# isds-neu/PeRCNN

Hardware: AMD Instinct MI355X
Metric: pi_block_rollout_fwd_bwd_steps_per_sec (higher is better)
Workload: dtype f32; 1 GPU; gs2d_512: gs2d 512x512, 2 species, Hc=8, T=1000 forward+backward rollout per step, dense dL/dtraj; reaction=poly, parallelism=single GPU, points=262144, T=1000

## Files before the change

### percnn_amd/csrc/pi_abi.hip

```cpp
#include <hip/hip_runtime.h>

#include <cstdint>
#include <cstdlib>
#include <chrono>
#include <cstdio>
#include <cstring>
#include <map>
#include <mutex>
#include <thread>
#include <tuple>
#include <vector>

#include "../../include/percnn_pi.h"
#include "pi_kernels.h"
#include "pi_tile2d.h"
#include "pi_stream3d.h"
#include "pi_brick3d.h"
#include "pi_res3d.h"
#include "pi_contract.h"
#include "pi_peer.h"
#include "pi_adv.h"
#include "pi_host.h"

namespace {

using pi::Geom;

struct Options {
    int block = 256;
    int vec = 0;
    int wgrad_blocks = 1024;
    int tile = 1;
    int tile_k = 4;
    int tile_nt = 512;
    int stream3d = 1;
    int tile_fuse = 1;
    int bwd_cpl = 2;
    int zc = 8;
    int overlap = 0;
    int overlap_chunk = 128;
    int fuse_wgrad = 2;
    int skip_wgrad = 0;
    int tile_xcd = 1;
    int tile_by = 0;
    int slab_fused_put_adj = 0;
    int peer_upb = 2048;
    int peer_upb_take = 0;
    int tile_persist = 2;
    int persist_handshake = 1;
    int fwd_small_half = 1;
    int adj_small_half = 1;
    int adj_small_pause = -1;
    int fwd_small_pause = -1;
    int persist_small = 1;
    int fwd_persist_per_cu = 1;
    int fwd_persist_f64 = 1;
    int adj_persist_f64 = 1;
    int fwd_persist = 1;
    int persist_split = 1;
    int persist_timeout_ms = 2000;
    int persist_first_timeout_ms = 100;
    int tile_wide = 3;
    int fwd_blocks = 0;
    int xcd_window = 0;
    int block_small = 1;
    int rz = 0;
// ... 990 lines not shown
    PI_TILE_DISPATCH(CALL_AT);
#undef CALL_AT
}

int device_cu_count()
{
    static int cu_count[16] = {};
    int dev = 0;
    if (hipGetDevice(&dev) != hipSuccess || dev < 0 || dev >= 16) return 0;
    if (!cu_count[dev]) {
        int n = 0;
        cu_count[dev] = (hipDeviceGetAttribute(&n, hipDeviceAttributeMultiprocessorCount, dev) == hipSuccess && n > 0) ? n : -1;
    }
    return cu_count[dev] > 0 ? cu_count[dev] : 0;
}

bool persist_disabled_here();
constexpr int PERSIST_BAND = 2 * (TILE_B * TILE_B - (TILE_B - 16) * (TILE_B - 16));
size_t persist_outbox_bytes(const Problem& p, int elem = 4)
{
    return (size_t)2 * (size_t)((p.n0 / TILE_B) * (p.W / TILE_B)) * PERSIST_BAND * (elem == 8 ? 16 : 8);
}

template <typename T>
bool persist_ok(const Problem& p, const unsigned char* mask, int t_top, int ngroups, hipStream_t st)
{
    if (!p.opt.tile_persist || ngroups < 2) return false;
    if (sizeof(T) != 4 && (!p.opt.adj_persist_f64 || !p.opt.persist_split)) return false;
    if (persist_disabled_here()) return false;
    if (mask && t_top >= 4096) return false;
    if (!tile_fuse_ok<T>(p) || tile_wide_for<T>(p, true) != 0 || tile_by_for(p) != TILE_B) return false;
    if (p.n0 % TILE_B || p.W % TILE_B) return false;
    const int64_t tiles = (p.n0 / TILE_B) * (p.W / TILE_B);
    const int cus = device_cu_count();
    if (tiles < 16 || cus <= 0 || tiles > cus) return false;
    hipStreamCaptureStatus cap = hipStreamCaptureStatusNone;
    if (hipStreamIsCapturing(st, &cap) != hipSuccess || cap != hipStreamCaptureStatusNone) return false;
    return true;
}

constexpr int PERSIST_SLOTS = 32;
struct PersistHost {
    volatile int slot[PERSIST_SLOTS][4];
};
struct PersistGuard {
    std::mutex mu;
// ... 294 lines not shown
    if (p.n0 % TILE_B || p.W % TILE_B) return false;
    const int64_t tiles = (p.n0 / TILE_B) * (p.W / TILE_B);
    const int cus = device_cu_count();
    if (tiles < 16 || cus <= 0 || tiles > (int64_t)cus * p.opt.fwd_persist_per_cu) return false;
    hipStreamCaptureStatus cap = hipStreamCaptureStatusNone;
    if (st && (hipStreamIsCapturing(st, &cap) != hipSuccess || cap != hipStreamCaptureStatusNone)) return false;
    return true;
}

template <typename T>
hipError_t launch_fwd_persist(T* frame_t0, int ngroups, const T* P, const Problem& p, hipStream_t st)
{
    constexpr int K = 4, NT = 512;
    pi_host::Resident r;
    if (!persist_enter(st, r.dev)) return hipErrorNotSupported;
    pi::TileGeom g = make_tile_geom(p, TILE_B);
    const unsigned grid = (unsigned)((p.n0 / TILE_B) * g.tiles_x);
    const size_t lds = pi::tile_state_bytes<T, K, TILE_B, TILE_B>() + (size_t)pi::PERSIST_SPLIT_TABLE_ROWS * NT * sizeof(int) + 16;
    const int two = (int64_t)grid > (int64_t)device_cu_count() ? 1 : 0;
    auto* k = two ? pi::pi_fwd2d_persist_kernel<T, K, TILE_B, TILE_B, NT, 2> : pi::pi_fwd2d_persist_kernel<T, K, TILE_B, TILE_B, NT, 1>;
    if (hipError_t e = allow_lds(k, lds)) return e;
    const int nb = persist_fits(k, NT, lds, r.dev);
    if (nb < 1 || (int64_t)grid > (int64_t)device_cu_count() * nb) return hipErrorCooperativeLaunchTooLarge;
    if (hipError_t e = persist_scratch(persist_outbox_bytes(p, (int)sizeof(T)), st, r)) return e;
    long frame_stride = (long)(2 * p.n);
    persist_claim(p.opt, r);
    pi::PersistArgs pa = persist_args(r, reinterpret_cast<unsigned long long*>(r.scratch + 256), reinterpret_cast<unsigned*>(r.scratch), ngroups);
    void* args[] = {(void*)&frame_t0, (void*)&frame_stride, (void*)&P, (void*)&g, (void*)&pa};
    hipError_t e;
    if (p.opt.tile_persist == 2) {
        hipLaunchKernelGGL(k, dim3(grid), dim3(NT), lds, st, frame_t0, frame_stride, P, g, pa);
        e = hipGetLastError();
    } else {
        e = hipLaunchCooperativeKernel(reinterpret_cast<const void*>(k), dim3(grid), dim3(NT), args, (unsigned)lds, st);
    }
    if (e != hipSuccess) return e;
    return persist_launched(st, r, p.opt.persist_handshake, grid, "the resident forward rollout");
}

int64_t persist_small_tiles(const Problem& p, int by) { return ((p.n0 + by - 1) / by) * ((p.W + TILE_B - 1) / TILE_B); }
size_t persist_small_outbox_bytes(const Problem& p, int elem)
{
    if (p.ndim != 2 || p.hc != 0 || elem != 4 || p.slab) return 0;
    const int by = tile_by_for(p);
    if (by >= TILE_B || persist_small_tiles(p, by) > 256) return 0;
    return align_up((size_t)2 * (size_t)persist_small_tiles(p, by) * (2 * TILE_B * by) * sizeof(unsigned long long), 256);
}

template <typename T>
bool persist_small_ok(const Problem& p, const unsigned char* mask, int t_top, int ngroups, hipStream_t st)
// ... 1678 lines not shown
    else           { if (vec == 1) PI_RSB(3, 1); else PI_RSB(3, V); }
#undef PI_RSB
    return (int)hipGetLastError();
}

}

namespace {

int apply_option(Options& o, const char* key, long value)
{
    if (!key) return PERCNN_PI_EINVAL;
    if (!std::strcmp(key, "vec")) {
        if (value != 0 && value != 1) return PERCNN_PI_EINVAL;
        o.vec = (int)value;
        return 0;
    }
    if (!std::strcmp(key, "tile")) {
        if (value < 0 || value > 2) return PERCNN_PI_EINVAL;
        o.tile = (int)value;
        return 0;
    }
    if (!std::strcmp(key, "tile_xcd")) { o.tile_xcd = value != 0; return 0; }
    if (!std::strcmp(key, "tile_by")) {
        if (value != 0 && value != 8 && value != 16 && value != 32) return PERCNN_PI_EINVAL;
        o.tile_by = (int)value;
        return 0;
    }
    if (!std::strcmp(key, "slab_fused_put_adj")) { o.slab_fused_put_adj = value != 0; return 0; }
    if (!std::strcmp(key, "peer_upb") || !std::strcmp(key, "peer_upb_take")) {
        const bool take = key[8] == '_';
        if ((value < 256 && !(take && value == 0)) || value > 65536) return PERCNN_PI_EINVAL;
        (take ? o.peer_upb_take : o.peer_upb) = (int)value;
        return 0;
    }
    if (!std::strcmp(key, "tile_persist")) {
        if (value < 0 || value > 2) return PERCNN_PI_EINVAL;
        o.tile_persist = (int)value;
        return 0;
    }
    if (!std::strcmp(key, "persist_handshake")) { o.persist_handshake = value != 0; return 0; }
    if (!std::strcmp(key, "persist_split")) { o.persist_split = value != 0; return 0; }
    if (!std::strcmp(key, "persist_small")) { if (value < 0 || value > 2) return PERCNN_PI_EINVAL; o.persist_small = (int)value; return 0; }
    if (!std::strcmp(key, "fwd_persist")) { o.fwd_persist = value != 0; return 0; }
    if (!std::strcmp(key, "fwd_persist_f64")) { o.fwd_persist_f64 = value != 0; return 0; }
    if (!std::strcmp(key, "adj_persist_f64")) { o.adj_persist_f64 = value != 0; return 0; }
// ... 272 lines not shown
    if (!traj || !out || nframes < 0 || out == traj || out == target) return PERCNN_PI_EINVAL;
    if (!ws || ws_bytes < (size_t)batch * batch_sqerr_slots(batch) * sizeof(double) || reinterpret_cast<uintptr_t>(ws) % 8)
        return PERCNN_PI_EWORKSPACE;
    return sample_sqerr<T>(traj, target, mask, nframes, p, batch, nullptr, scale, out, ws, static_cast<hipStream_t>(stream));
}

template <typename T>
int batch_obs_sqerr_impl(const T* traj, const T* target_c, const unsigned char* mask, int nframes, int ndim, const int64_t* shape,
                         const int* strides, int batch, double scale, T* out, void* ws, size_t ws_bytes, void* stream)
{
    if (batch < 1 || batch > MAX_BATCH) return PERCNN_PI_EINVAL;
    Problem p;
    if (int rc = batch_problem(0, ndim, shape, batch, p, nullptr, false)) return rc;
    if (!traj || !out || nframes < 0 || out == traj || out == target_c) return PERCNN_PI_EINVAL;
    ObsHost oh;
    if (int rc = make_obs(p, batch, strides, target_c, mask, nframes, oh)) return rc;
    if (!ws || ws_bytes < (size_t)batch * batch_sqerr_slots(batch) * sizeof(double) || reinterpret_cast<uintptr_t>(ws) % 8)
        return PERCNN_PI_EWORKSPACE;
    return sample_sqerr<T>(traj, target_c, mask, nframes, p, batch, &oh, scale, out, ws, static_cast<hipStream_t>(stream));
}
}

namespace {
template <typename T>
int debug_plan_impl(int hc, int ndim, const int64_t* shape, const char* options, int* out)
{
    Problem p;
    if (int rc = make_problem(hc, ndim, shape, false, p, options, false)) return rc;
    const int vec = pick_vec<T>(p, {});
    auto family = [&](bool adjoint, bool wgrad, int& planes) {
        planes = 1;
        if (p.hc == -1) return 4;
        if (tile_eligible<T>(p, {}, adjoint)) return 1;
        if (!adjoint || !wgrad || (p.hc == 0 && sizeof(T) == 4))
            if (stream3d_vec<T>(p, {}, adjoint)) return 2;
        if (!adjoint || !wgrad || p.hc == 0)
            if (const int brz = brick_rz_for<T>(p, vec, adjoint)) { planes = brz; return 3; }
        planes = direct_rz<T>(p, vec, adjoint);
        return 0;
    };
    const bool f32poly = hc == 0 && sizeof(T) == 4;
    const bool tiled_adj = tile_eligible<T>(p, {}, true);
    const bool direct_sweep = !tiled_adj && (f32poly || !stream3d_vec<T>(p, {}, true));
    const bool tile_fused = tiled_adj && tile_fuse_ok<T>(p);
    const bool fuse = tile_fused || (direct_sweep && !p.opt.skip_wgrad && hc != -1 &&
                                     (p.opt.fuse_wgrad == 1 || (p.opt.fuse_wgrad == 2 && hc == 0)));
    const int K = (p.opt.tile_k == 8 && p.hc != 0) ? 4 : p.opt.tile_k;
    out[0] = family(false, false, out[5]);
    out[1] = family(true, fuse, out[6]);
    out[2] = fuse ? 1 : 0;
    out[3] = out[0] == 1 ? K : 1;
// ... 21 lines not shown
    }
    return 0;
}

template <typename T>
int debug_batch_plan_impl(int hc, int ndim, const int64_t* shape, int batch, const char* options, int* out)
{
    if (batch == 1) {
        int o[32] = {};
        if (int rc = debug_plan_impl<T>(hc, ndim, shape, options, o)) return rc;
        out[0] = o[0]; out[1] = o[1]; out[2] = o[5]; out[3] = o[6];
        return 0;
    }
    Problem p;
    if (int rc = batch_problem(hc, ndim, shape, batch, p, options, false)) return rc;
    const int vec = pick_vec<T>(p, {});
    const bool fuse = !p.opt.skip_wgrad && (p.opt.fuse_wgrad == 1 || (p.opt.fuse_wgrad == 2 && hc == 0));
    const int fz = batch_brick_rz<T>(p, vec, batch, false, false, false), az = batch_brick_rz<T>(p, vec, batch, true, fuse, false);
    out[0] = fz ? 3 : 0; out[1] = az ? 3 : 0;
    out[2] = fz ? fz : 1; out[3] = az ? az : 1;
    return 0;
}

}

namespace pi_host {
int resident_async_error() { return persist_async_error(); }
int resident_cu_count() { return device_cu_count(); }
hipError_t resident_begin(void* stream, size_t outbox_bytes, Resident& r)
{
    auto st = static_cast<hipStream_t>(stream);
    Options o;
    { std::lock_guard<std::mutex> lk(g_defaults_mu); o = g_defaults; }
    if (!o.tile_persist || !o.fwd_persist) return hipErrorNotSupported;
    hipStreamCaptureStatus cap = hipStreamCaptureStatusNone;
    if (hipStreamIsCapturing(st, &cap) != hipSuccess || cap != hipStreamCaptureStatusNone) { (void)hipGetLastError(); return hipErrorNotSupported; }
    if (!persist_enter(st, r.dev)) return hipErrorNotSupported;
    if (hipError_t e = persist_scratch(outbox_bytes, st, r)) return e;
    persist_claim(o, r);
    return hipSuccess;
}
hipError_t resident_launched(void* stream, Resident& r, unsigned grid, const char* what)
{
    int handshake;
    { std::lock_guard<std::mutex> lk(g_defaults_mu); handshake = g_defaults.persist_handshake; }
    return persist_launched(static_cast<hipStream_t>(stream), r, handshake, grid, what);
// ... 66 lines not shown
    Problem p;
    if (int rc = make_problem(0, ndim, shape, false, p, options)) return rc;
    if (!out || (elem_size != 4 && elem_size != 8)) return PERCNN_PI_EINVAL;
    const int vec = (p.W % (16 / elem_size) == 0 && p.opt.vec != 1) ? 16 / elem_size : 1;
    Geom g = make_geom(p);
    const int block = direct_block(p, g, vec);
    const int rz = elem_size == 4 ? direct_rz<float>(p, vec, true) : direct_rz<double>(p, vec, true);
    if (!set_blockmap(g, p.ndim, vec, block, (size_t)elem_size, p.opt.l2_tile_kb * 1024, rz, (long)p.opt.l2_tile_min_kb * 1024,
                      p.opt.lane_x)) return PERCNN_PI_EINVAL;
    out[0] = g.lxs; out[1] = g.nxb; out[2] = g.nrg; out[3] = (int)g.nblk; out[4] = rz; out[5] = block;
    return 0;
}

int percnn_pi_debug_batch_plan(int hc, int ndim, const int64_t* shape, int elem_size, int batch, const char* options, int* out)
{
    if (!out || (elem_size != 4 && elem_size != 8)) return PERCNN_PI_EINVAL;
    return elem_size == 4 ? debug_batch_plan_impl<float>(hc, ndim, shape, batch, options, out)
                          : debug_batch_plan_impl<double>(hc, ndim, shape, batch, options, out);
}

int percnn_pi_debug_plan(int hc, int ndim, const int64_t* shape, int elem_size, const char* options, int* out)
{
    if (!out || (elem_size != 4 && elem_size != 8)) return PERCNN_PI_EINVAL;
    return elem_size == 4 ? debug_plan_impl<float>(hc, ndim, shape, options, out) : debug_plan_impl<double>(hc, ndim, shape, options, out);
}

size_t percnn_pi_param_count(int hc) { return hc < -1 ? 0 : (size_t)pi::nparams(hc); }

#define PI_CONTRACT(SUF, T)                                                                                             \
    int percnn_pi_contract_fwd_##SUF(const T* params, int hc, T* poly, void* stream)                                   \
    {                                                                                                                   \
        if (!params || !poly || hc < 1) return PERCNN_PI_EINVAL;                                                        \
        hipLaunchKernelGGL((pi::pi_contract_fwd_kernel<T>), dim3(1), dim3(128), 0, static_cast<hipStream_t>(stream),    \
                           params, hc, poly);                                                                           \
        return (int)hipGetLastError();                                                                                  \
    }                                                                                                                   \
    int percnn_pi_contract_bwd_##SUF(const T* params, int hc, const T* g_poly, T* g_params, void* stream)              \
    {                                                                                                                   \
        if (!params || !g_poly || !g_params || hc < 1) return PERCNN_PI_EINVAL;                                         \
        hipLaunchKernelGGL((pi::pi_contract_bwd_kernel<T>), dim3(1), dim3(256), 0, static_cast<hipStream_t>(stream),   \
                           params, hc, g_poly, g_params);                                                               \
        return (int)hipGetLastError();                                                                                  \
    }
PI_CONTRACT(f32, float)
PI_CONTRACT(f64, double)
#undef PI_CONTRACT

// ... 53 lines not shown
{
    Problem p;
    if (make_problem(hc, ndim, shape, false, p, nullptr, false) || (elem_size != 4 && elem_size != 8)) return 0;
    Problem q = p;
    q.n = (p.n0 + 4) * p.n1 * p.W;
    return workspace_bytes(q, elem_size);
}

size_t percnn_pi_rollout_bwd_workspace_bytes(int hc, int ndim, const int64_t* shape, int T_steps, int elem_size)
{
    Problem p;
    if (make_problem(hc, ndim, shape, false, p, nullptr, false) || (elem_size != 4 && elem_size != 8) || T_steps < 0) return 0;
    size_t need = rollout_workspace_bytes(p, T_steps, elem_size);
    for (int by : {8, 16}) {
        Problem q = p;
        q.opt.tile_by = by;
        need = std::max(need, rollout_workspace_bytes(q, T_steps, elem_size));
    }
    return need;
}

int percnn_pi_set_option(const char* key, long value)
{
    std::lock_guard<std::mutex> lk(g_defaults_mu);
    return apply_option(g_defaults, key, value);
}

int percnn_pi_host_words_alloc(void** p, size_t bytes)
{
    if (!p || bytes == 0) return PERCNN_PI_EINVAL;
    void* hp = nullptr;
    if (hipError_t e = hipHostMalloc(&hp, bytes, hipHostMallocMapped | hipHostMallocCoherent)) return (int)e;
    std::memset(hp, 0, bytes);
    *p = hp;
    return 0;
}
int percnn_pi_host_words_free(void* p) { return p ? (int)hipHostFree(p) : 0; }

namespace {
__global__ void pi_debug_hog_kernel(unsigned long long ticks, int* started)
{
    extern __shared__ unsigned char hog_lds[];
    hog_lds[threadIdx.x] = (unsigned char)threadIdx.x;
    if (threadIdx.x == 0 && started) __hip_atomic_store(started + blockIdx.x, 1, __ATOMIC_RELAXED, __HIP_MEMORY_SCOPE_SYSTEM);
    const unsigned long long t0 = wall_clock64();
    while (wall_clock64() - t0 < ticks) __builtin_amdgcn_s_sleep(64);
// ... 360 lines not shown
```

### percnn_amd/csrc/pi_tile2d.h

```cpp
#pragma once
#include <type_traits>
#include "pi_device.h"

namespace pi {

#ifdef PI_TILE_TIMING
__device__ long long pi_tile_stamps[4096 * 16];
__device__ long long pi_tile_wave_stamps[256 * 16 * 16];
#define PI_STAMP(i) do { if (threadIdx.x == 0) pi_tile_stamps[blockIdx.x * 16 + (i)] = wall_clock64();                      \
                         if (threadIdx.x % 64 == 0 && blockIdx.x < 256)                                                      \
                             pi_tile_wave_stamps[(blockIdx.x * 16 + threadIdx.x / 64) * 16 + (i)] = wall_clock64(); } while (0)
#define PI_STAMP_PREV() do { if (threadIdx.x == 0) pi_tile_stamps[blockIdx.x * 16 + 14] = pi_tile_stamps[blockIdx.x * 16 + 15]; } while (0)
#else
#define PI_STAMP(i) do { } while (0)
#define PI_STAMP_PREV() do { } while (0)
#endif

#ifdef PI_PERSIST_STAMPS
__device__ long long pi_persist_stamps[256 * 8 * 16];
#define PI_PSTAMP(i) do { if (grp == PI_PERSIST_STAMPS && threadIdx.x % 64 == 0 && blockIdx.x < 256)                      \
                              pi_persist_stamps[(blockIdx.x * 8 + threadIdx.x / 64) * 16 + (i)] = wall_clock64(); } while (0)
#else
#define PI_PSTAMP(i) do { } while (0)
#endif
// ... 14 lines not shown
    return ((size_t)4 * Tile<K, BX, BY>::PLANE * sizeof(T) + 32 + 15) / 16 * 16;
}

__device__ __forceinline__ void lds_add_f64(double* p, double v)
{
    (void)__hip_atomic_fetch_add(p, v, __ATOMIC_RELAXED, __HIP_MEMORY_SCOPE_WORKGROUP);
}

struct TileGeom {
    int H, W;
    long ss;
    int tiles_x;
    int rx, rw, rh;
    LossInj loss;
};

__device__ __forceinline__ int tile_of_block(int b, const TileGeom& g)
{
    if (g.rx == 0) return b;
    const int xcd = b % NXCD, j = b / NXCD;
    const int ty = (xcd / g.rx) * g.rh + j / g.rw, tx = (xcd % g.rx) * g.rw + j % g.rw;
    return ty * g.tiles_x + tx;
}

__device__ __forceinline__ int wrap1(int g, int n) { return g < 0 ? g + n : (g >= n ? g - n : g); }

template <typename T> struct lds_pad0 { static constexpr int value = sizeof(T) == 4 ? 2 : 0; };
template <typename T> struct lds_pad1 { static constexpr int value = sizeof(T) == 4 ? 4 : 0; };

template <typename T, int K, int BX, int BY, int NT>
struct WindowLoader {
    using TL = Tile<K, BX, BY>;
    static constexpr int VEC = vec_width<T>::value;
    static constexpr int LXV = TL::LX / VEC;
    static constexpr int N = 2 * TL::LY * LXV;
    static constexpr int TRIPS = (N + NT - 1) / NT;
    Pack<T, VEC> p[TRIPS];
    int dst[TRIPS];
    __device__ __forceinline__ void issue(const T* __restrict__ src, const TileGeom& g, int ty0, int tx0)
    {
#pragma unroll
        for (int q = 0; q < TRIPS; ++q) {
            const int i = threadIdx.x + q * NT;
            dst[q] = -1;
            if (i < N) {
                const int s = i / (TL::LY * LXV);
// ... 1068 lines not shown
    if (has_slot) {
        double sum = 0.0;
        if (threadIdx.x < 2) {
            for (int w = 0; w < NW; ++w) sum += red[w * 2 + threadIdx.x];
        } else if constexpr (MOM) {
            sum = red[2 * NW + threadIdx.x - 2];
        }
        *pslot = pold + sum;
    }
    PI_STAMP(15);
}

struct PersistArgs {
    unsigned long long* outbox;
    unsigned* sync;
    int* host;
    int ngroups;
    unsigned long long timeout_ticks;
    unsigned long long first_timeout_ticks;
    int t_top;
    int pause;
    int masked;
    unsigned frames[128];
};

template <int K>
__device__ __forceinline__ unsigned persist_mask(const PersistArgs& pa, int t)
{
    if (!pa.masked) return (1u << K) - 1u;
    unsigned m = 0;
#pragma unroll
    for (int q = 0; q < K; ++q) {
        const int f = t - 1 - q;
        m |= ((pa.frames[f >> 5] >> (f & 31)) & 1u) << q;
    }
    return m;
}

template <int B, int HW>
__device__ __forceinline__ int band_index(int y, int x)
{
    if (y < HW) return y * B + x;
    if (y >= B - HW) return HW * B + (y - (B - HW)) * B + x;
    const int r = y - HW;
    return 2 * HW * B + r * 2 * HW + (x < HW ? x : HW + (x - (B - HW)));
}
// ... 180 lines not shown
        double a0 = 0.0, a1 = 0.0, a2 = 0.0, a3 = 0.0;
#pragma unroll
        for (int k = 0; k < NT; k += 64) {
            const double v0 = row[k], v1 = row[k + 16], v2 = row[k + 32], v3 = row[k + 48];
            a0 += v0; a1 += v1; a2 += v2; a3 += v3;
        }
        double a = (a0 + a1) + (a2 + a3);
        a += dpp_mov<0x111, 0xF>(a);
        a += dpp_mov<0x112, 0xF>(a);
        a += dpp_mov<0x114, 0xF>(a);
        a += dpp_mov<0x118, 0xF>(a);
        if (part == 15) partials[(long)blockIdx.x * np + P_W + mm] += a;
    }
}


typedef unsigned pi_v4u __attribute__((ext_vector_type(4)));
template <typename T> struct GranuleIO;
template <> struct GranuleIO<float> {
    using Raw = pi_v4u;
    static constexpr int BYTES = 16, VALS = 2;
    __amdgpu_buffer_rsrc_t rs;
    __device__ __forceinline__ GranuleIO(void* outbox, size_t bytes) : rs(__builtin_amdgcn_make_buffer_rsrc(outbox, 0, (int)bytes, 0x00020000)) {}
    __device__ __forceinline__ void put(size_t idx, unsigned epoch, const float* src) const
    {
        const Pack<float, 2> v = ld<float, 2>(src);
        const pi_v4u w = {__builtin_bit_cast(unsigned, v.v[0]), epoch, __builtin_bit_cast(unsigned, v.v[1]), epoch};
        __builtin_amdgcn_raw_buffer_store_b128(w, rs, (int)(idx * 16), 0,  16);
    }
    __device__ __forceinline__ Raw get(size_t idx) const { return __builtin_amdgcn_raw_buffer_load_b128(rs, (int)(idx * 16), 0, 16); }
    static __device__ __forceinline__ bool ok(Raw x, unsigned epoch) { return x.y == epoch && x.w == epoch; }
    static __device__ __forceinline__ void land(Raw x, float* dst)
    {
        const unsigned a = x.x, b = x.z;
        st<float, 2>(dst, Pack<float, 2>{{__builtin_bit_cast(float, a), __builtin_bit_cast(float, b)}});
    }
};
template <> struct GranuleIO<double> {
    using Raw = pi_v4u;
    static constexpr int BYTES = 16, VALS = 1;
    __amdgpu_buffer_rsrc_t rs;
    __device__ __forceinline__ GranuleIO(void* outbox, size_t bytes) : rs(__builtin_amdgcn_make_buffer_rsrc(outbox, 0, (int)bytes, 0x00020000)) {}
    __device__ __forceinline__ void put(size_t idx, unsigned epoch, const double* src) const
    {
        const unsigned long long b = __builtin_bit_cast(unsigned long long, *src);
        const pi_v4u w = {(unsigned)b, epoch, (unsigned)(b >> 32), epoch};
        __builtin_amdgcn_raw_buffer_store_b128(w, rs, (int)(idx * 16), 0,  16);
    }
    __device__ __forceinline__ Raw get(size_t idx) const { return __builtin_amdgcn_raw_buffer_load_b128(rs, (int)(idx * 16), 0, 16); }
    static __device__ __forceinline__ bool ok(Raw x, unsigned epoch) { return x.y == epoch && x.w == epoch; }
    static __device__ __forceinline__ void land(Raw x, double* dst) { *dst = __builtin_bit_cast(double, ((unsigned long long)x.z << 32) | x.x); }
};

template <typename T, bool PAIRS> struct SmallGranule {
    using Raw = unsigned long long;
    static __device__ __forceinline__ bool ok(Raw x, unsigned epoch) { return (unsigned)(x >> 32) == epoch; }
    static __device__ __forceinline__ void land(Raw x, T* dst) { *dst = __builtin_bit_cast(T, (unsigned)x); }
};
template <typename T> struct SmallGranule<T, true> {
    using Raw = typename GranuleIO<T>::Raw;
    static __device__ __forceinline__ bool ok(Raw x, unsigned epoch) { return GranuleIO<T>::ok(x, epoch); }
    static __device__ __forceinline__ void land(Raw x, T* dst) { GranuleIO<T>::land(x, dst); }
};
template <typename T, int K, int BX, int BY, int NT, bool HALFS = false>
__global__ void __launch_bounds__(NT)
pi_adj2d_persist_small_kernel(const T* __restrict__ hframe_t, const T* __restrict__ gframe_t, T* __restrict__ aframe_t,
                              long frame_stride, T* __restrict__ g_h0, double* __restrict__ partials, int np,
                              const T* __restrict__ P_in, TileGeom g, PersistArgs pa)
{
    static_assert(sizeof(T) == 4 && K % 2 == 0, "float32; an even number of sub-steps leaves the state in buffer 0");
// ... 99 lines not shown
        adj_substeps<T, POLY, K, BX, BY, NT, 0, PRE, false, true, HALFS>(b0, b1, hframe_t + go, gframe_t + go, aframe_t + go,
                                                                         frame_stride, gmask, g_h0, g_h0 && last ? K : 0, g, ty0,
                                                                         tx0, P, acc_c, ops0, mom, sa, nullptr, last, tab_geo, &jp,
                                                                         hoff);
        if (last) break;
        const long gn = go - (long)K * frame_stride;
        gmask = persist_mask<K>(pa, pa.t_top - K * (grp + 1));
        if constexpr (HALFS)
            persist_load_ops_half<T>(ops0, hframe_t + gn - frame_stride, gmask & 1u ? gframe_t + gn - frame_stride : nullptr, g, hoff[0]);
        else if constexpr (PRE)
            adj_load_ops<T, K, BX, BY, NT, 0>(ops0, 0, hframe_t + gn - frame_stride, gmask & 1u ? gframe_t + gn - frame_stride : nullptr, g,
                                              ty0, tx0, &sa[0]);
        const unsigned epoch = (unsigned)grp + 1u;
        gu64* half = outbox + (size_t)(epoch & 1u) * (size_t)ntiles * (2 * OWN);
        gu64* mine = half + (size_t)tile * (2 * OWN);
        const size_t halfu = (size_t)(epoch & 1u) * (size_t)ntiles * (2 * OWN / GV);
#pragma unroll
        for (int q = 0; q < NPUB; ++q) {
            const int i = (int)threadIdx.x + q * NT;
            if (i < 2 * OWN / GV) {
                const int sp = i / (OWN / GV), e = (i - sp * (OWN / GV)) * GV, y = e / BX, x = e - y * BX;
                const T* src = b0 + sp * TL::PLANE + (HW + y) * LXW + HW + x;
                if constexpr (PAIRS) {
                    gio.put(halfu + (size_t)tile * (2 * OWN / GV) + (size_t)i, epoch, src);
                } else {
                    const unsigned v = __builtin_bit_cast(unsigned, *src);
                    __hip_atomic_store(mine + i, ((unsigned long long)epoch << 32) | v, __ATOMIC_RELAXED, __HIP_MEMORY_SCOPE_AGENT);
                }
            }
        }
        tile_store<T, K, BX, BY, NT, true>(b0, aframe_t + gn, g, ty0, tx0);
        for (int w = 0; w < pa.pause; ++w) __builtin_amdgcn_s_sleep(1);
        int gl[NGAT], gs[NGAT];
        typename SmallGranule<T, PAIRS>::Raw gx[NGAT];
        auto fetch = [&](int idx) {
            if constexpr (PAIRS) return gio.get(halfu + (size_t)idx);
            else return __hip_atomic_load(half + idx, __ATOMIC_RELAXED, __HIP_MEMORY_SCOPE_AGENT);
        };
#pragma unroll
        for (int q = 0; q < NGAT; ++q) {
            gl[q] = tab_gl[q * NT + (int)threadIdx.x];
            gs[q] = tab_gs[q * NT + (int)threadIdx.x];
            gx[q] = fetch(gs[q]);
        }
        const unsigned long long t0 = wall_clock64();
        const unsigned long long bound = grp == 0 ? pa.first_timeout_ticks : pa.timeout_ticks;
        for (;;) {
// ... 75 lines not shown
    o.ju[0] = a2.v[0]; o.ju[1] = a2.v[1]; o.ju[2] = b2.v[0]; o.ju[3] = b2.v[1];
    o.jv[0] = c2.v[0]; o.jv[1] = c2.v[1]; o.jv[2] = d2.v[0]; o.jv[3] = d2.v[1];
}

template <int K, int BX, int GV, int NT>
struct HandOver {
    using TL = Tile<K, BX, BX>;
    static constexpr int HW = 2 * K, LXW = TL::LX;
    static constexpr int BANDH = BX * BX - (BX - 2 * HW) * (BX - 2 * HW);
    static constexpr int RINGH = LXW * LXW - BX * BX;
    static_assert(BANDH % GV == 0 && RINGH % GV == 0 && HW % GV == 0 && BX % GV == 0, "granules of x-adjacent values");
    static constexpr int BANDU = BANDH / GV, RINGU = RINGH / GV;
    static constexpr int NPUB = (2 * BANDU + NT - 1) / NT, NGAT = (2 * RINGU + NT - 1) / NT;
    static __device__ __forceinline__ int pub_pos(int i)
    {
        if (i >= 2 * BANDU) return -1;
        const int sp = i / BANDU, e = (i - sp * BANDU) * GV;
        int y, x;
        if (e < HW * BX) { y = e / BX; x = e - y * BX; }
        else if (e < 2 * HW * BX) { const int m = e - HW * BX; y = BX - HW + m / BX; x = m % BX; }
        else { const int m = e - 2 * HW * BX; y = HW + m / (2 * HW); const int c = m % (2 * HW); x = c < HW ? c : BX - 2 * HW + c; }
        return sp * TL::PLANE + (HW + y) * LXW + HW + x;
    }
    static __device__ __forceinline__ void gat_pos(int r, const TileGeom& g, int ty0, int tx0, int tiles_y, int& gl, int& gs)
    {
        gl = -1; gs = 0;
        if (r >= 2 * RINGU) return;
        const int sp = r / RINGU, e = (r - sp * RINGU) * GV;
        int wy, wx;
        if (e < HW * LXW) { wy = e / LXW; wx = e - wy * LXW; }
        else if (e < HW * LXW + BX * 2 * HW) { const int m = e - HW * LXW; wy = HW + m / (2 * HW); const int c = m % (2 * HW); wx = c < HW ? c : BX + c; }
        else { const int m = e - HW * LXW - BX * 2 * HW; wy = HW + BX + m / LXW; wx = m % LXW; }
        const int gy = ty0 + wy - HW, gx = tx0 + wx - HW;
        const int nty = ((gy + g.H) / BX) % tiles_y, ntx = ((gx + g.W) / BX) % g.tiles_x;
        const int ly = (gy + g.H) % BX, lx = (gx + g.W) % BX;
        gl = sp * TL::PLANE + wy * LXW + wx;
        gs = (nty * g.tiles_x + ntx) * (2 * BANDU) + sp * BANDU + band_index<BX, HW>(ly, lx) / GV;
    }
};

constexpr int PERSIST_SPLIT_TABLE_ROWS = 19;

template <typename T, int PASS> struct sweep_half_pass {
    static constexpr int HALF_PASS_MASK = 0x39;
    static constexpr bool value = PASS != 2 && ((HALF_PASS_MASK >> PASS) & 1) != 0;
};
constexpr int SWEEP_HALF_P5_SPLIT = 128;

template <int PASS> struct PersistPass;
template <> struct PersistPass<0> { static constexpr int M1 = 0, P1 = PART_PYR, SPLIT = 1 << 30, M2 = 0, P2 = PART_PYR; };
template <> struct PersistPass<1> { static constexpr int M1 = 1, P1 = PART_PYR, SPLIT = 1 << 30, M2 = 1, P2 = PART_PYR; };
template <> struct PersistPass<2> { static constexpr int M1 = 2, P1 = PART_PYR, SPLIT = 128, M2 = 0, P2 = PART_ANN; };
template <> struct PersistPass<3> { static constexpr int M1 = 1, P1 = PART_ANN, SPLIT = 1 << 30, M2 = 1, P2 = PART_ANN; };
template <> struct PersistPass<4> { static constexpr int M1 = 2, P1 = PART_ANN, SPLIT = 1 << 30, M2 = 2, P2 = PART_ANN; };
template <> struct PersistPass<5> { static constexpr int M1 = 3, P1 = PART_PYR, SPLIT = 64, M2 = 3, P2 = PART_ANN; };

template <typename T, int K, int BX, int BY, int NT, int PASS>
__device__ __forceinline__ StripOff persist_pass_off(const TileGeom& g, int ty0, int tx0, bool upper)
{
    using PP = PersistPass<PASS>;
    StripOff so;
    if constexpr (PP::SPLIT >= NT) {
// ... 253 lines not shown
        if constexpr (sizeof(T) == 4) {
            if ((grp & 3) == 3 || last) {
#pragma unroll
                for (int s = 0; s < 2; ++s)
#pragma unroll
                    for (int m = 0; m < 10; ++m) {
                        double* slot = lacc + (10 * s + m) * NT + (int)threadIdx.x;
                        *slot += (double)mom_total(mom.a[s][m]);
                        mom.a[s][m] = V2<T>{T(0), T(0)};
                    }
            }
        }
        if (last) {
            T* dst = g_h0 ? g_h0 : aframe_t - (long)(grp + 1) * K * frame_stride;
            tile_store<T, K, BX, BY, NT, true>(b0, dst, g, ty0, tx0);
            break;
        }
        gmask = gmask_next;
        const unsigned ep1 = (unsigned)grp + 1u;
        const size_t mine = (size_t)(ep1 & 1u) * (size_t)ntiles * (2 * BANDU) + (size_t)tile * (2 * BANDU);
#pragma unroll
        for (int q = 0; q < NPUB; ++q) {
            const int pl = tab_pub[q * NT + (int)threadIdx.x];
            if (pl >= 0) gio.put(mine + (size_t)((int)threadIdx.x + q * NT), ep1, b0 + pl);
        }
        PI_PSTAMP(8);
    }

    lds_barrier();
    double* red = reinterpret_cast<double*>(smem_raw);
    constexpr int NW = NT / WAVE;
    const int wave = threadIdx.x / WAVE, lane = threadIdx.x % WAVE;
#pragma unroll
    for (int s = 0; s < 2; ++s) {
        const double r = wave_sum_to_last(acc_c[s]);
        if (lane == REDUCE_LANE) red[s * NW + wave] = r;
    }
    lds_barrier();
    if (threadIdx.x < 2) {
        double sum = 0.0;
        for (int w = 0; w < NW; ++w) sum += red[(int)threadIdx.x * NW + w];
        partials[(long)blockIdx.x * np + P_COEF + (int)threadIdx.x] += sum;
    }
    if (threadIdx.x < 320) {
        const int mm = (int)threadIdx.x >> 4, part = (int)threadIdx.x & 15;
        const double* row = lacc + mm * LACC + part;
        double a0 = 0.0, a1 = 0.0, a2 = 0.0, a3 = 0.0;
// ... 157 lines not shown
    using TL = Tile<K, BX, BY>;
    using HO = HandOver<K, BX, GranuleIO<T>::VALS, NT>;
    constexpr int BANDU = HO::BANDU, NPUB = HO::NPUB, NGAT = HO::NGAT;
    static_assert(NPUB + 2 * NGAT <= 13, "tables fit the LDS the host reserves");
    constexpr int IDLE = 4 * WAVE;
    extern __shared__ __attribute__((aligned(16))) unsigned char smem_raw[];
    T* b0 = reinterpret_cast<T*>(smem_raw) + lds_pad0<T>::value;
    T* b1 = reinterpret_cast<T*>(smem_raw) + 2 * TL::PLANE + lds_pad1<T>::value;
    const int tile = tile_of_block(blockIdx.x, g);
    const int tyi = tile / g.tiles_x, txi = tile % g.tiles_x, tiles_y = g.H / BY;
    const int ty0 = tyi * BY, tx0 = txi * BX;
    const int ntiles = g.tiles_x * tiles_y;
    const GranuleIO<T> gio(pa.outbox, (size_t)2 * (size_t)ntiles * (2 * BANDU) * GranuleIO<T>::BYTES);

    int* tab_pub = reinterpret_cast<int*>(smem_raw + tile_state_bytes<T, K, BX, BY>());
    int* tab_gl = tab_pub + NPUB * NT;
    int* tab_gs = tab_gl + NGAT * NT;
    unsigned* tab_geo = reinterpret_cast<unsigned*>(tab_pub + 13 * NT);
    int* wg_abort = tab_pub + PERSIST_SPLIT_TABLE_ROWS * NT;
    if (threadIdx.x == 0) {
        *wg_abort = 0;
        const unsigned n = __hip_atomic_fetch_add(pa.sync, 1u, __ATOMIC_RELAXED, __HIP_MEMORY_SCOPE_AGENT) + 1u;
        if (n == (unsigned)ntiles && pa.host) __hip_atomic_store(pa.host, 1, __ATOMIC_RELAXED, __HIP_MEMORY_SCOPE_SYSTEM);
    }
    tab_geo[0 * NT + (int)threadIdx.x] = persist_pass_geo<K, BX, BY, NT, 0>(g, ty0, tx0);
    tab_geo[1 * NT + (int)threadIdx.x] = persist_pass_geo<K, BX, BY, NT, 1>(g, ty0, tx0);
    tab_geo[2 * NT + (int)threadIdx.x] = persist_pass_geo<K, BX, BY, NT, 2>(g, ty0, tx0);
    tab_geo[3 * NT + (int)threadIdx.x] = persist_pass_geo<K, BX, BY, NT, 3>(g, ty0, tx0);
    tab_geo[4 * NT + (int)threadIdx.x] = persist_pass_geo<K, BX, BY, NT, 4>(g, ty0, tx0);
    tab_geo[5 * NT + (int)threadIdx.x] = persist_pass_geo<K, BX, BY, NT, 5>(g, ty0, tx0);
#pragma unroll
    for (int q = 0; q < NPUB; ++q) tab_pub[q * NT + (int)threadIdx.x] = HO::pub_pos((int)threadIdx.x + q * NT);
#pragma unroll
    for (int q = 0; q < NGAT; ++q) {
        int gl, gs;
        HO::gat_pos((int)threadIdx.x + q * NT, g, ty0, tx0, tiles_y, gl, gs);
        tab_gl[q * NT + (int)threadIdx.x] = gl;
        tab_gs[q * NT + (int)threadIdx.x] = gs;
    }
    tile_load<T, K, BX, BY, NT>(frames, g, ty0, tx0, b0);
    __syncthreads();
    const int tid = (int)threadIdx.x;
    static_assert(HOLDP == 1 || HOLDP == 2, "the parameter block is held in vector or in scalar registers");
    T Ph[NPOLY];
    unsigned gw[7];
    FwdStoreMap<T, K, BX, BY, NT, IDLE> smap;
    FwdStoreMap<T, K, BX, BY, NT, 0> smap_all;
    const int wave_id = __builtin_amdgcn_readfirstlane(tid >> 6);
#pragma unroll
    for (int i = 0; i < NPOLY; ++i) {
        T x = P_in[i];
        if constexpr (HOLDP == 2) asm volatile("" : "+s"(x));
        else asm volatile("" : "+v"(x));
        Ph[i] = x;
    }
// ... 83 lines not shown
        else { half_strip(b0, b1, gw[2]); half_strip(b0, b1, gw[6]); }
        lds_barrier();
        PI_PSTAMP(4);
        smap_all.template store<false, 2>(b1, fr + frame_stride);
        PI_PSTAMP(9);
        half_strip(b1, b0, gw[3]);
        PI_PSTAMP(10);
        lds_barrier();
        PI_PSTAMP(5);
        smap_all.template store<true, 0>(b0, fr + 2 * frame_stride);
        half_strip(b0, b1, gw[4]);
        lds_barrier();
        PI_PSTAMP(6);
        smap_all.template store<false, 0>(b1, fr + 3 * frame_stride);
        half_strip(b1, b0, gw[5]);
        lds_barrier();
        PI_PSTAMP(7);
        if (grp + 1 == pa.ngroups) {
            tile_store<T, K, BX, BY, NT, true>(b0, fr + (long)K * frame_stride, g, ty0, tx0);
            break;
        }
        const unsigned ep1 = (unsigned)grp + 1u;
        const size_t mine = (size_t)(ep1 & 1u) * (size_t)ntiles * (2 * BANDU) + (size_t)tile * (2 * BANDU);
#pragma unroll
        for (int q = 0; q < NPUB; ++q) {
            const int pl = tab_pub[q * NT + tid];
            if (pl >= 0) gio.put(mine + (size_t)(tid + q * NT), ep1, b0 + pl);
        }
        PI_PSTAMP(8);
    }
}

template <typename T, int K, int BX, int BY, int NT, bool HALFS = false>
__global__ void __launch_bounds__(NT)
pi_fwd2d_persist_small_kernel(T* __restrict__ frames , long frame_stride,
                              const T* __restrict__ P_in, TileGeom g, PersistArgs pa)
{
    static_assert(sizeof(T) == 4 && K % 2 == 0, "float32; an even number of sub-steps leaves the state in buffer 0");
    using TL = Tile<K, BX, BY>;
    constexpr int HW = 2 * K, LXW = TL::LX, LYW = TL::LY;
    constexpr int OWN = BX * BY;
    constexpr int RINGH = LXW * LYW - OWN;
    constexpr bool PAIRS = HALFS && GranuleIO<T>::VALS == 2;
    constexpr int GV = PAIRS ? 2 : 1;
    static_assert(OWN % (2 * GV) == 0 && RINGH % GV == 0 && BX % GV == 0 && HW % GV == 0, "granules of x-adjacent values");
    constexpr int NPUB = (2 * OWN / GV + NT - 1) / NT, NGAT = (2 * RINGH / GV + NT - 1) / NT;
    extern __shared__ __attribute__((aligned(16))) unsigned char smem_raw[];
    T* b0 = reinterpret_cast<T*>(smem_raw) + lds_pad0<T>::value;
    T* b1 = reinterpret_cast<T*>(smem_raw) + 2 * TL::PLANE + lds_pad1<T>::value;
    const int tile = tile_of_block(blockIdx.x, g);
// ... 60 lines not shown
        gw[3] = fwd_half_word<K, BX, BY, 3, PART_FULL>(tid);
#pragma unroll
        for (int m = 0; m < K; ++m) asm volatile("" : "+v"(gw[m]));
    }
    for (int grp = 0; grp < pa.ngroups; ++grp) {
        T* fr = frames + (long)grp * K * frame_stride;
        const bool last = grp + 1 == pa.ngroups;
        fwd_substeps<T, POLY, K, BX, BY, NT, 0, false, GEO, WT, HALFS>(b0, b1, fr, frame_stride, g, ty0, tx0, P, HALFS ? gw : tab_geo);
        if (last) {
            tile_store<T, K, BX, BY, NT, true, WT>(b0, fr + (long)K * frame_stride, g, ty0, tx0);
            break;
        }
        const unsigned epoch = (unsigned)grp + 1u;
        gu64* half = outbox + (size_t)(epoch & 1u) * (size_t)ntiles * (2 * OWN);
        gu64* mine = half + (size_t)tile * (2 * OWN);
        const size_t halfu = (size_t)(epoch & 1u) * (size_t)ntiles * (2 * OWN / GV);
#pragma unroll
        for (int q = 0; q < NPUB; ++q) {
            const int i = tid + q * NT;
            if (i < 2 * OWN / GV) {
                const int sp = i / (OWN / GV), e = (i - sp * (OWN / GV)) * GV, y = e / BX, x = e - y * BX;
                const T* src = b0 + sp * TL::PLANE + (HW + y) * LXW + HW + x;
                if constexpr (PAIRS) {
                    gio.put(halfu + (size_t)tile * (2 * OWN / GV) + (size_t)i, epoch, src);
                } else {
                    const unsigned v = __builtin_bit_cast(unsigned, *src);
                    __hip_atomic_store(mine + i, ((unsigned long long)epoch << 32) | v, __ATOMIC_RELAXED, __HIP_MEMORY_SCOPE_AGENT);
                }
            }
        }
        tile_store<T, K, BX, BY, NT, true, WT>(b0, fr + (long)K * frame_stride, g, ty0, tx0);
        for (int w = 0; w < pa.pause; ++w) __builtin_amdgcn_s_sleep(1);
        int gl[NGAT], gs[NGAT];
        typename SmallGranule<T, PAIRS>::Raw gx[NGAT];
        auto fetch = [&](int idx) {
            if constexpr (PAIRS) return gio.get(halfu + (size_t)idx);
            else return __hip_atomic_load(half + idx, __ATOMIC_RELAXED, __HIP_MEMORY_SCOPE_AGENT);
        };
#pragma unroll
        for (int q = 0; q < NGAT; ++q) {
            gl[q] = tab_gl[q * NT + tid];
            gs[q] = tab_gs[q * NT + tid];
            gx[q] = fetch(gs[q]);
        }
        const unsigned long long t0 = wall_clock64();
        const unsigned long long bound = grp == 0 ? pa.first_timeout_ticks : pa.timeout_ticks;
        bool failed = false;
// ... 37 lines not shown
```

Baseline: 327,300 steps/s.

## Use non-bypassing stores for halo hand-over when all readers share the XCD

In the persistent forward rollout kernel, each tile writes its XCC id into a small scratch table at startup. On the first group it checks which neighbouring tiles run on the same XCD. Halo granules read only by same-XCD neighbours are then stored with default cache policy instead of the cache-bypassing bit, so they can stay in the shared L2 rather than going out to far memory. This relies on the readers landing on the expected XCD and adds a debug query path; a wrong locality guess would risk stale reads.

```diff
diff --git a/percnn_amd/csrc/pi_abi.hip b/percnn_amd/csrc/pi_abi.hip
--- a/percnn_amd/csrc/pi_abi.hip
+++ b/percnn_amd/csrc/pi_abi.hip
@@ -42,6 +42,8 @@
     int fuse_wgrad = 2;
     int skip_wgrad = 0;
     int tile_xcd = 1;
+    int handover_local = 1;
+    int debug_handover_local = 0;
     int tile_by = 0;
     int slab_fused_put_adj = 0;
     int peer_upb = 2048;
@@ -1078,6 +1080,8 @@
     return (size_t)2 * (size_t)((p.n0 / TILE_B) * (p.W / TILE_B)) * PERSIST_BAND * (elem == 8 ? 16 : 8);
 }
 
+size_t persist_xcc_bytes(const Problem& p) { return align_up((size_t)((p.n0 / TILE_B) * (p.W / TILE_B)) * sizeof(unsigned), 16); }
+
 template <typename T>
 bool persist_ok(const Problem& p, const unsigned char* mask, int t_top, int ngroups, hipStream_t st)
 {
@@ -1418,10 +1422,12 @@
     if (hipError_t e = allow_lds(k, lds)) return e;
     const int nb = persist_fits(k, NT, lds, r.dev);
     if (nb < 1 || (int64_t)grid > (int64_t)device_cu_count() * nb) return hipErrorCooperativeLaunchTooLarge;
-    if (hipError_t e = persist_scratch(persist_outbox_bytes(p, (int)sizeof(T)), st, r)) return e;
+    const size_t outbox_bytes = persist_outbox_bytes(p, (int)sizeof(T));
+    if (hipError_t e = persist_scratch(outbox_bytes + persist_xcc_bytes(p), st, r)) return e;
     long frame_stride = (long)(2 * p.n);
     persist_claim(p.opt, r);
     pi::PersistArgs pa = persist_args(r, reinterpret_cast<unsigned long long*>(r.scratch + 256), reinterpret_cast<unsigned*>(r.scratch), ngroups);
+    if (p.opt.handover_local) pa.xcc = reinterpret_cast<unsigned*>(r.scratch + 256 + outbox_bytes);
     void* args[] = {(void*)&frame_t0, (void*)&frame_stride, (void*)&P, (void*)&g, (void*)&pa};
     hipError_t e;
     if (p.opt.tile_persist == 2) {
@@ -3146,6 +3152,12 @@
         return 0;
     }
     if (!std::strcmp(key, "tile_xcd")) { o.tile_xcd = value != 0; return 0; }
+    if (!std::strcmp(key, "handover_local")) { o.handover_local = value != 0; return 0; }
+    if (!std::strcmp(key, "debug_handover_local")) {
+        if (value < 0 || value > (1 << 24)) return PERCNN_PI_EINVAL;
+        o.debug_handover_local = (int)value;
+        return 0;
+    }
     if (!std::strcmp(key, "tile_by")) {
         if (value != 0 && value != 8 && value != 16 && value != 32) return PERCNN_PI_EINVAL;
         o.tile_by = (int)value;
@@ -3464,11 +3476,13 @@
 }
 
 namespace {
-template <typename T>
-int debug_plan_impl(int hc, int ndim, const int64_t* shape, const char* options, int* out)
+int debug_handover_local(const Problem& p, int elem_size, int* out);
+template <typename T>
+int debug_plan_impl(int hc, int ndim, const int64_t* shape, const char* options, int* out, bool query_ok = false)
 {
     Problem p;
     if (int rc = make_problem(hc, ndim, shape, false, p, options, false)) return rc;
+    if (p.opt.debug_handover_local) return query_ok ? debug_handover_local(p, (int)sizeof(T), out) : (int)PERCNN_PI_EINVAL;
     const int vec = pick_vec<T>(p, {});
     auto family = [&](bool adjoint, bool wgrad, int& planes) {
         planes = 1;
@@ -3536,6 +3550,28 @@
     return 0;
 }
 
+int debug_handover_local(const Problem& p, int elem_size, int* out)
+{
+    if (p.ndim != 2 || p.n0 % TILE_B || p.W % TILE_B) return PERCNN_PI_EINVAL;
+    const pi::TileGeom g = make_tile_geom(p, TILE_B);
+    const int tiles_y = (int)(p.n0 / TILE_B);
+    auto bitmaps = [&](auto ho) {
+        using HO = decltype(ho);
+        static_assert(2 * HO::BANDU % 32 == 0, "whole bitmap words per tile");
+        constexpr int WORDS = 2 * HO::BANDU / 32;
+        if ((int64_t)tiles_y * g.tiles_x * WORDS > (int64_t)p.opt.debug_handover_local) return (int)PERCNN_PI_EINVAL;
+        for (int ty = 0; ty < tiles_y; ++ty)
+            for (int tx = 0; tx < g.tiles_x; ++tx) {
+                int* w = out + (size_t)(ty * g.tiles_x + tx) * WORDS;
+                for (int i = 0; i < WORDS; ++i) w[i] = 0;
+                for (int i = 0; i < 2 * HO::BANDU; ++i)
+                    if (p.opt.handover_local && HO::pub_local(i, g, ty, tx, tiles_y)) w[i / 32] |= (int)(1u << (i % 32));
+            }
+        return 0;
+    };
+    return elem_size == 4 ? bitmaps(pi::HandOver<4, TILE_B, 2, 512>{}) : bitmaps(pi::HandOver<4, TILE_B, 1, 512>{});
+}
+
 }
 
 namespace pi_host {
@@ -3648,7 +3684,7 @@
 int percnn_pi_debug_plan(int hc, int ndim, const int64_t* shape, int elem_size, const char* options, int* out)
 {
     if (!out || (elem_size != 4 && elem_size != 8)) return PERCNN_PI_EINVAL;
-    return elem_size == 4 ? debug_plan_impl<float>(hc, ndim, shape, options, out) : debug_plan_impl<double>(hc, ndim, shape, options, out);
+    return elem_size == 4 ? debug_plan_impl<float>(hc, ndim, shape, options, out, true) : debug_plan_impl<double>(hc, ndim, shape, options, out, true);
 }
 
 size_t percnn_pi_param_count(int hc) { return hc < -1 ? 0 : (size_t)pi::nparams(hc); }
@@ -3748,6 +3784,7 @@
 
 int percnn_pi_set_option(const char* key, long value)
 {
+    if (key && !std::strcmp(key, "debug_handover_local")) return PERCNN_PI_EINVAL;
     std::lock_guard<std::mutex> lk(g_defaults_mu);
     return apply_option(g_defaults, key, value);
 }
diff --git a/percnn_amd/csrc/pi_tile2d.h b/percnn_amd/csrc/pi_tile2d.h
--- a/percnn_amd/csrc/pi_tile2d.h
+++ b/percnn_amd/csrc/pi_tile2d.h
@@ -60,6 +60,7 @@
     const int ty = (xcd / g.rx) * g.rh + j / g.rw, tx = (xcd % g.rx) * g.rw + j % g.rw;
     return ty * g.tiles_x + tx;
 }
+__host__ __device__ __forceinline__ int xcd_of_tile(int ty, int tx, const TileGeom& g) { return (ty / g.rh) * g.rx + tx / g.rw; }
 
 __device__ __forceinline__ int wrap1(int g, int n) { return g < 0 ? g + n : (g >= n ? g - n : g); }
 
@@ -1174,6 +1175,7 @@
     int pause;
     int masked;
     unsigned frames[128];
+    unsigned* xcc;
 };
 
 template <int K>
@@ -1400,11 +1402,12 @@
     static constexpr int BYTES = 16, VALS = 2;
     __amdgpu_buffer_rsrc_t rs;
     __device__ __forceinline__ GranuleIO(void* outbox, size_t bytes) : rs(__builtin_amdgcn_make_buffer_rsrc(outbox, 0, (int)bytes, 0x00020000)) {}
-    __device__ __forceinline__ void put(size_t idx, unsigned epoch, const float* src) const
+    __device__ __forceinline__ void put(size_t idx, unsigned epoch, const float* src, bool local) const
     {
         const Pack<float, 2> v = ld<float, 2>(src);
         const pi_v4u w = {__builtin_bit_cast(unsigned, v.v[0]), epoch, __builtin_bit_cast(unsigned, v.v[1]), epoch};
-        __builtin_amdgcn_raw_buffer_store_b128(w, rs, (int)(idx * 16), 0,  16);
+        if (local) __builtin_amdgcn_raw_buffer_store_b128(w, rs, (int)(idx * 16), 0,  0);
+        else __builtin_amdgcn_raw_buffer_store_b128(w, rs, (int)(idx * 16), 0,  16);
     }
     __device__ __forceinline__ Raw get(size_t idx) const { return __builtin_amdgcn_raw_buffer_load_b128(rs, (int)(idx * 16), 0, 16); }
     static __device__ __forceinline__ bool ok(Raw x, unsigned epoch) { return x.y == epoch && x.w == epoch; }
@@ -1419,11 +1422,12 @@
     static constexpr int BYTES = 16, VALS = 1;
     __amdgpu_buffer_rsrc_t rs;
     __device__ __forceinline__ GranuleIO(void* outbox, size_t bytes) : rs(__builtin_amdgcn_make_buffer_rsrc(outbox, 0, (int)bytes, 0x00020000)) {}
-    __device__ __forceinline__ void put(size_t idx, unsigned epoch, const double* src) const
+    __device__ __forceinline__ void put(size_t idx, unsigned epoch, const double* src, bool local) const
     {
         const unsigned long long b = __builtin_bit_cast(unsigned long long, *src);
         const pi_v4u w = {(unsigned)b, epoch, (unsigned)(b >> 32), epoch};
-        __builtin_amdgcn_raw_buffer_store_b128(w, rs, (int)(idx * 16), 0,  16);
+        if (local) __builtin_amdgcn_raw_buffer_store_b128(w, rs, (int)(idx * 16), 0,  0);
+        else __builtin_amdgcn_raw_buffer_store_b128(w, rs, (int)(idx * 16), 0,  16);
     }
     __device__ __forceinline__ Raw get(size_t idx) const { return __builtin_amdgcn_raw_buffer_load_b128(rs, (int)(idx * 16), 0, 16); }
     static __device__ __forceinline__ bool ok(Raw x, unsigned epoch) { return x.y == epoch && x.w == epoch; }
@@ -1569,7 +1573,7 @@
                 const int sp = i / (OWN / GV), e = (i - sp * (OWN / GV)) * GV, y = e / BX, x = e - y * BX;
                 const T* src = b0 + sp * TL::PLANE + (HW + y) * LXW + HW + x;
                 if constexpr (PAIRS) {
-                    gio.put(halfu + (size_t)tile * (2 * OWN / GV) + (size_t)i, epoch, src);
+                    gio.put(halfu + (size_t)tile * (2 * OWN / GV) + (size_t)i, epoch, src,  false);
                 } else {
                     const unsigned v = __builtin_bit_cast(unsigned, *src);
                     __hip_atomic_store(mine + i, ((unsigned long long)epoch << 32) | v, __ATOMIC_RELAXED, __HIP_MEMORY_SCOPE_AGENT);
@@ -1691,6 +1695,46 @@
         else { const int m = e - 2 * HW * BX; y = HW + m / (2 * HW); const int c = m % (2 * HW); x = c < HW ? c : BX - 2 * HW + c; }
         return sp * TL::PLANE + (HW + y) * LXW + HW + x;
     }
+    static __host__ __device__ __forceinline__ int pub_readers(int i)
+    {
+        const int e = (i % BANDU) * GV;
+        int y, x;
+        if (e < HW * BX) { y = e / BX; x = e - y * BX; }
+        else if (e < 2 * HW * BX) { const int m = e - HW * BX; y = BX - HW + m / BX; x = m % BX; }
+        else { const int m = e - 2 * HW * BX; y = HW + m / (2 * HW); const int c = m % (2 * HW); x = c < HW ? c : BX - 2 * HW + c; }
+        const int dy = y < HW ? -1 : (y >= BX - HW ? 1 : 0), dx = x < HW ? -1 : (x >= BX - HW ? 1 : 0);
+        int r = 0;
+        if (dy) r |= 1 << ((dy + 1) * 3 + 1);
+        if (dx) r |= 1 << (3 + dx + 1);
+        if (dy && dx) r |= 1 << ((dy + 1) * 3 + dx + 1);
+        return r;
+    }
+    static __host__ __device__ __forceinline__ int same_xcd(const TileGeom& g, int tyi, int txi, int tiles_y)
+    {
+        if (g.rx == 0) return 0;
+        const int me = xcd_of_tile(tyi, txi, g);
+        int r = 0;
+        for (int dy = -1; dy <= 1; ++dy)
+            for (int dx = -1; dx <= 1; ++dx) {
+                if (!dy && !dx) continue;
+                const int ny = (tyi + dy + tiles_y) % tiles_y, nx = (txi + dx + g.tiles_x) % g.tiles_x;
+                if (xcd_of_tile(ny, nx, g) == me) r |= 1 << ((dy + 1) * 3 + dx + 1);
+            }
+        return r;
+    }
+    static __host__ __device__ __forceinline__ bool pub_local(int i, const TileGeom& g, int tyi, int txi, int tiles_y)
+    {
+        return (pub_readers(i) & ~same_xcd(g, tyi, txi, tiles_y)) == 0;
+    }
+    static constexpr int PUB_POS = 0xFFFF, PUB_READERS = 0x1FF, PUB_NEVER = 1 << 4, PUB_LOCAL = 1 << 30;
+    static_assert(2 * TL::PLANE <= PUB_POS, "an LDS position fits the low half of a table entry");
+    static __device__ __forceinline__ int pub_entry(int i, int same)
+    {
+        const int pl = pub_pos(i);
+        if (pl < 0) return -1;
+        const int rd = pub_readers(i);
+        return pl | ((rd & ~same) == 0 ? rd : PUB_NEVER) << 16;
+    }
     static __device__ __forceinline__ void gat_pos(int r, const TileGeom& g, int ty0, int tx0, int tiles_y, int& gl, int& gs)
     {
         gl = -1; gs = 0;
@@ -1707,6 +1751,35 @@
         gs = (nty * g.tiles_x + ntx) * (2 * BANDU) + sp * BANDU + band_index<BX, HW>(ly, lx) / GV;
     }
 };
+
+__device__ __forceinline__ unsigned handover_xcc_word()
+{
+    return 0x80000000u | (unsigned)__builtin_amdgcn_s_getreg( 20 | (3 << 11));
+}
+__device__ __forceinline__ void handover_announce(const PersistArgs& pa, int tile)
+{
+    if (pa.xcc) __hip_atomic_store(pa.xcc + tile, handover_xcc_word(), __ATOMIC_RELAXED, __HIP_MEMORY_SCOPE_AGENT);
+}
+template <typename HO, int NT>
+__device__ __forceinline__ void handover_confirm(const PersistArgs& pa, const TileGeom& g, int tyi, int txi, int tiles_y, int* tab_pub)
+{
+    int ok = 0;
+    if (pa.xcc) {
+        const unsigned me = handover_xcc_word();
+#pragma unroll
+        for (int b = 0; b < 9; ++b) {
+            if (b == 4) continue;
+            const int ny = (tyi + b / 3 - 1 + tiles_y) % tiles_y, nx = (txi + b % 3 - 1 + g.tiles_x) % g.tiles_x;
+            const unsigned w = __hip_atomic_load(pa.xcc + ny * g.tiles_x + nx, __ATOMIC_RELAXED, __HIP_MEMORY_SCOPE_AGENT);
+            ok |= (w == me ? 1 : 0) << b;
+        }
+    }
+#pragma unroll
+    for (int q = 0; q < HO::NPUB; ++q) {
+        const int e = tab_pub[q * NT + (int)threadIdx.x];
+        if (e >= 0) tab_pub[q * NT + (int)threadIdx.x] = (e & HO::PUB_POS) | ((((e >> 16) & HO::PUB_READERS) & ~ok) == 0 ? HO::PUB_LOCAL : 0);
+    }
+}
 
 constexpr int PERSIST_SPLIT_TABLE_ROWS = 19;
 
@@ -2006,7 +2079,7 @@
 #pragma unroll
         for (int q = 0; q < NPUB; ++q) {
             const int pl = tab_pub[q * NT + (int)threadIdx.x];
-            if (pl >= 0) gio.put(mine + (size_t)((int)threadIdx.x + q * NT), ep1, b0 + pl);
+            if (pl >= 0) gio.put(mine + (size_t)((int)threadIdx.x + q * NT), ep1, b0 + pl,  false);
         }
         PI_PSTAMP(8);
     }
@@ -2210,6 +2283,7 @@
         *wg_abort = 0;
         const unsigned n = __hip_atomic_fetch_add(pa.sync, 1u, __ATOMIC_RELAXED, __HIP_MEMORY_SCOPE_AGENT) + 1u;
         if (n == (unsigned)ntiles && pa.host) __hip_atomic_store(pa.host, 1, __ATOMIC_RELAXED, __HIP_MEMORY_SCOPE_SYSTEM);
+        handover_announce(pa, tile);
     }
     tab_geo[0 * NT + (int)threadIdx.x] = persist_pass_geo<K, BX, BY, NT, 0>(g, ty0, tx0);
     tab_geo[1 * NT + (int)threadIdx.x] = persist_pass_geo<K, BX, BY, NT, 1>(g, ty0, tx0);
@@ -2217,8 +2291,9 @@
     tab_geo[3 * NT + (int)threadIdx.x] = persist_pass_geo<K, BX, BY, NT, 3>(g, ty0, tx0);
     tab_geo[4 * NT + (int)threadIdx.x] = persist_pass_geo<K, BX, BY, NT, 4>(g, ty0, tx0);
     tab_geo[5 * NT + (int)threadIdx.x] = persist_pass_geo<K, BX, BY, NT, 5>(g, ty0, tx0);
-#pragma unroll
-    for (int q = 0; q < NPUB; ++q) tab_pub[q * NT + (int)threadIdx.x] = HO::pub_pos((int)threadIdx.x + q * NT);
+    const int same = pa.xcc ? HO::same_xcd(g, tyi, txi, tiles_y) : 0;
+#pragma unroll
+    for (int q = 0; q < NPUB; ++q) tab_pub[q * NT + (int)threadIdx.x] = HO::pub_entry((int)threadIdx.x + q * NT, same);
 #pragma unroll
     for (int q = 0; q < NGAT; ++q) {
         int gl, gs;
@@ -2348,10 +2423,11 @@
         }
         const unsigned ep1 = (unsigned)grp + 1u;
         const size_t mine = (size_t)(ep1 & 1u) * (size_t)ntiles * (2 * BANDU) + (size_t)tile * (2 * BANDU);
+        if (grp == 0) handover_confirm<HO, NT>(pa, g, tyi, txi, tiles_y, tab_pub);
 #pragma unroll
         for (int q = 0; q < NPUB; ++q) {
             const int pl = tab_pub[q * NT + tid];
-            if (pl >= 0) gio.put(mine + (size_t)(tid + q * NT), ep1, b0 + pl);
+            if (pl >= 0) gio.put(mine + (size_t)(tid + q * NT), ep1, b0 + (pl & HO::PUB_POS), (pl & HO::PUB_LOCAL) != 0);
         }
         PI_PSTAMP(8);
     }
@@ -2458,7 +2534,7 @@
                 const int sp = i / (OWN / GV), e = (i - sp * (OWN / GV)) * GV, y = e / BX, x = e - y * BX;
                 const T* src = b0 + sp * TL::PLANE + (HW + y) * LXW + HW + x;
                 if constexpr (PAIRS) {
-                    gio.put(halfu + (size_t)tile * (2 * OWN / GV) + (size_t)i, epoch, src);
+                    gio.put(halfu + (size_t)tile * (2 * OWN / GV) + (size_t)i, epoch, src,  false);
                 } else {
                     const unsigned v = __builtin_bit_cast(unsigned, *src);
                     __hip_atomic_store(mine + i, ((unsigned long long)epoch << 32) | v, __ATOMIC_RELAXED, __HIP_MEMORY_SCOPE_AGENT);
```

Measured after the change: 337,300 steps/s (median of 6 runs). 1.03x the previous value.
